# vita-epfl/collaborative-gan-sampling

Measured on AMD Instinct MI355X. Metric: refined samples/sec @ 20 refinement steps, higher is better.
Workload: dtype f32; 1 GPU; dcgan64 collaborative refinement (propose + K-step refine + render), batch 1024/GPU, K=20, momentum rate 0.1, refine at feature [8, 8, 256], random-init weights, z~U(-1,1) seed 2019+rank; global_batch=1024, refine_steps=20, parallelism=single GPU, hipgraph=True, batches_in_flight=2, fused_per_launch=1, sync_bn=False, contraction=f32

## Files before the change

collaborative-gan-sampling_amd/csrc/bn.hip:

```cpp
#include "cgs_internal.h"

#define BN_MAX_BLOCKS CGS_BN_MAX_BLOCKS

struct BnGeom {
    int G;
    int rows_per_block;
};

static BnGeom bn_geom(int M, int C) {
    BnGeom g;
    int rpb = cgs_ceil_div(M, BN_MAX_BLOCKS);
    if (rpb < 16) rpb = 16;
    g.rows_per_block = rpb;
    g.G = cgs_ceil_div(M, rpb);
    (void)C;
    return g;
}

size_t cgs_bn_ws_bytes(int M, int C) {
    (void)M;
    return ((size_t)BN_MAX_BLOCKS * 2 * C + 6 * (size_t)C) * sizeof(float);
}

__device__ __forceinline__ void bn_affine4(const float* __restrict__ mean, const float* __restrict__ invstd, const float* __restrict__ gamma,
// ... 388 lines not shown
        }
    }
    __syncthreads();
    if (!live) return;
    const float4 s0 = bc[0][q], s1 = bc[1][q];
    const int r0 = blockIdx.y * rows_per_block, r1 = min(M, r0 + rows_per_block);
    const size_t base = (size_t)grp * M * C + c;
    if (!BWD) {
        const float4 g = *(const float4*)(gamma + c), bt = *(const float4*)(beta + c);
        float4 sc, sh;
        sc.x = g.x * s1.x; sc.y = g.y * s1.y; sc.z = g.z * s1.z; sc.w = g.w * s1.w;
        sh.x = bt.x - s0.x * sc.x; sh.y = bt.y - s0.y * sc.y; sh.z = bt.z - s0.z * sc.z; sh.w = bt.w - s0.w * sc.w;
        for (int r = r0 + rl; r < r1; r += 16) {
            const float4 v = *(const float4*)(x + base + (size_t)r * C);
            float4 o;
            o.x = fmaf(v.x, sc.x, sh.x); o.y = fmaf(v.y, sc.y, sh.y); o.z = fmaf(v.z, sc.z, sh.z); o.w = fmaf(v.w, sc.w, sh.w);
            o.x = o.x > 0.f ? o.x : leak * o.x; o.y = o.y > 0.f ? o.y : leak * o.y;
            o.z = o.z > 0.f ? o.z : leak * o.z; o.w = o.w > 0.f ? o.w : leak * o.w;
            *(float4*)(out + base + (size_t)r * C) = o;
        }
    } else {
        float4 mean, inv, sc, sh;
        bn_affine4(mean_io + (size_t)grp * C, invstd_io + (size_t)grp * C, gamma, beta, c, mean, inv, sc, sh);
        const float4 m1 = s0, m2 = s1;
        for (int r = r0 + rl; r < r1; r += 16) {
            const float4 xv = *(const float4*)(x + base + (size_t)r * C), dv = *(const float4*)(dy + base + (size_t)r * C);
            float4 o;
            BWD1(x) BWD1(y) BWD1(z) BWD1(w)
            *(float4*)(out + base + (size_t)r * C) = o;
        }
    }
}

#undef BWD1

static int norm_fa_rows_per_block(int groups, int rows_per_seg, int nseg, int M_group, int C) {
    const long max_rows = 16;
    const size_t max_bytes = (size_t)2 << 20;
    if ((long)rows_per_seg * nseg > max_rows || (long)rows_per_seg * nseg > NFA_MAX_ROWS || groups > 65535) return 0;
    if ((size_t)groups * M_group * C * sizeof(float) > max_bytes) return 0;
    const long cg = cgs_ceil_div(C, 64);
    long chunks = 1024 / ((long)groups * cg);
    if (chunks < 1) chunks = 1;
    long rpb = cgs_ceil_div(M_group, (int)chunks);
    if (rpb < 16) rpb = 16;
    rpb = (rpb + 15) / 16 * 16;
    if (cgs_ceil_div(M_group, (int)rpb) > 65535) return 0;
    return (int)rpb;
}

int cgs_bn_train_lrelu_fwd(const float* x, const float* gamma, const float* beta, float eps, float leak, float* y,
                           float* mean, float* invstd, int M, int C, void* ws, size_t ws_bytes, void* stream) {
    if (M <= 0 || C <= 0 || (C & 3)) return cgs_set_error(CGS_EINVAL, "bn fwd: M=%d C=%d (C must be a multiple of 4)", M, C);
    if (ws_bytes < cgs_bn_ws_bytes(M, C)) return cgs_set_error(CGS_EWORKSPACE, "bn fwd: workspace %zu < %zu", ws_bytes, cgs_bn_ws_bytes(M, C));
    hipStream_t s = (hipStream_t)stream;
    if (norm_small_ok(M)) {
        hipLaunchKernelGGL(norm_small_kernel<false>, dim3(cgs_ceil_div(C, 64), 1), dim3(256), 0, s, x, nullptr, gamma, beta, eps, leak, y, mean, invstd, nullptr, M, C);
        CGS_CHECK_LAUNCH("bn_train_lrelu_fwd");
        return CGS_OK;
    }
    const BnGeom g = bn_geom(M, C);
    float* part = (float*)ws;
    float* stat = part + (size_t)BN_MAX_BLOCKS * 2 * C;
    hipLaunchKernelGGL(bn_partial_kernel<0>, dim3(g.G), dim3(256), 0, s, x, nullptr, nullptr, nullptr, nullptr, nullptr, leak, part, M, C, g.rows_per_block);
    hipLaunchKernelGGL(bn_finalize_kernel<0>, dim3(cgs_ceil_div(C, BNF_CH)), dim3(256), 0, s, part, g.G, M, C, gamma, beta, eps, stat, mean, invstd);
    const size_t n4 = (size_t)M * C / 4;
    hipLaunchKernelGGL(bn_apply_fwd_kernel, dim3(ew_blocks(n4)), dim3(256), 0, s, x, stat, leak, y, n4, C, n4);
    CGS_CHECK_LAUNCH("bn_train_lrelu_fwd");
// ... 237 lines not shown

int cgs_norm_lrelu_bwd_from_partials(const float* dy, const float* x, const float* part, int groups, int rows_per_seg, int nseg, int seg_stride,
                                     const float* gamma, const float* beta, const float* mean, const float* invstd, float leak, float* dx,
                                     int M_group, int C, void* ws, size_t ws_bytes, void* stream) {
    if (groups <= 0 || groups > 65535 || M_group <= 0 || C <= 0 || (C & 3) || rows_per_seg <= 0 || nseg <= 0 || seg_stride < 0 || !part || !dy || !x || !dx)
        return cgs_set_error(CGS_EINVAL, "norm bwd from partials: groups=%d M=%d C=%d rows=%d x %d", groups, M_group, C, rows_per_seg, nseg);
    const bool sliced = groups == 1 && nseg == 1 && rows_per_seg >= 1024 && !((uintptr_t)ws & 7);
    const size_t need = (size_t)groups * 2 * C * sizeof(float) + (sliced ? (size_t)BNF_SLICES * 2 * C * sizeof(double) : 0);
    if (!ws || ws_bytes < need) return cgs_set_error(CGS_EWORKSPACE, "norm bwd from partials: workspace %zu < %zu", ws_bytes, need);
    hipStream_t s = (hipStream_t)stream;
    if (const int rpb = norm_fa_rows_per_block(groups, rows_per_seg, nseg, M_group, C)) {
        hipLaunchKernelGGL(norm_fa_kernel<true>, dim3(cgs_ceil_div(C, 64), cgs_ceil_div(M_group, rpb), groups), dim3(256), 0, s, x, dy, part, rows_per_seg, nseg,
                           seg_stride, gamma, beta, 0.f, leak, dx, (float*)mean, (float*)invstd, M_group, C, rpb);
        CGS_CHECK_LAUNCH("norm_lrelu_bwd_from_partials");
        return CGS_OK;
    }
    float* stat2;
    if (sliced) {
        double* slices = (double*)ws;
        stat2 = (float*)(slices + (size_t)BNF_SLICES * 2 * C);
        hipLaunchKernelGGL(bn_slice_sums_kernel, dim3(cgs_ceil_div(C, BNF_CH), BNF_SLICES), dim3(256), 0, s, part, rows_per_seg, C, slices);
        hipLaunchKernelGGL(bn_finalize2_slices_kernel, dim3(cgs_ceil_div(C, 64)), dim3(64), 0, s, slices, M_group, C, stat2);
    } else {
        stat2 = (float*)ws;
        hipLaunchKernelGGL(bn_finalize_kernel<1>, dim3(cgs_ceil_div(C, BNF_CH), groups), dim3(256), 0, s, part, rows_per_seg, M_group, C, nullptr, nullptr, 0.f,
                           stat2, nullptr, nullptr, nseg, seg_stride);
    }
    const size_t n4 = (size_t)groups * M_group * C / 4, gn4 = (size_t)M_group * C / 4;
    hipLaunchKernelGGL(bn_apply_bwd_kernel, dim3(ew_blocks(n4)), dim3(256), 0, s, dy, x, mean, invstd, gamma, beta, stat2, leak, dx, n4, C, gn4);
    CGS_CHECK_LAUNCH("norm_lrelu_bwd_from_partials");
    return CGS_OK;
}

int cgs_instnorm_lrelu_bwd_data(const float* dy, const float* x, const float* scale, const float* offset, const float* mean,
                                const float* invstd, float leak, float* dx, int B, int HW, int C, void* ws, size_t ws_bytes,
                                void* stream) {
    if (B <= 0 || HW <= 0 || C <= 0 || (C & 3) || B > 65535) return cgs_set_error(CGS_EINVAL, "instnorm bwd: B=%d HW=%d C=%d", B, HW, C);
    if (ws_bytes < cgs_instnorm_ws_bytes(B, HW, C)) return cgs_set_error(CGS_EWORKSPACE, "instnorm bwd: workspace %zu < %zu", ws_bytes, cgs_instnorm_ws_bytes(B, HW, C));
    hipStream_t s = (hipStream_t)stream;
    const BnGeom g = in_geom(B, HW);
    float* part = (float*)ws;
    float* stat = part + (size_t)B * g.G * 2 * C;
    float* stat2 = stat + (size_t)B * 4 * C;
    if (norm_small_ok(HW)) {
        hipLaunchKernelGGL(norm_small_kernel<true>, dim3(cgs_ceil_div(C, 64), B), dim3(256), 0, s, x, dy, scale, offset, 0.f, leak, dx, (float*)mean, (float*)invstd, stat2, HW, C);
        CGS_CHECK_LAUNCH("instnorm_lrelu_bwd_data");
        return CGS_OK;
    }
    hipLaunchKernelGGL(bn_partial_kernel<1>, dim3(g.G, B), dim3(256), 0, s, x, dy, mean, invstd, scale, offset, leak, part, HW, C, g.rows_per_block);
    hipLaunchKernelGGL(bn_finalize_kernel<1>, dim3(cgs_ceil_div(C, BNF_CH), B), dim3(256), 0, s, part, g.G, HW, C, nullptr, nullptr, 0.f, stat2, nullptr, nullptr);
    const size_t n4 = (size_t)B * HW * C / 4, gn4 = (size_t)HW * C / 4;
    hipLaunchKernelGGL(bn_apply_bwd_kernel, dim3(ew_blocks(n4)), dim3(256), 0, s, dy, x, mean, invstd, scale, offset, stat2, leak, dx, n4, C, gn4);
    CGS_CHECK_LAUNCH("instnorm_lrelu_bwd_data");
    return CGS_OK;
}
```

collaborative-gan-sampling_amd/engine.py:

```python
import gc

import numpy as np
import torch

from . import kernels as K
from . import lib as L
from .nets import ARCHS, _same_out, g_input_shape, layer_ks


class _Stage:
    out = None
    bwd_epi = (L.EPI_NONE, None, None)
    pre_folded = False
    bwd_nstat = None
    bstat = None

    def fwd(self, x):
        raise NotImplementedError

    def bwd(self, dy):
        raise NotImplementedError


class _View(_Stage):
# ... 107 lines not shown
        return K.linear_bwd_data(dy, self.w, out=self.dx)


class _BnTrainLrelu(_Stage):

    def __init__(self, B, shape, gamma, beta, leak, dev):
        self.gamma, self.beta, self.leak = gamma, beta, leak
        self.out = torch.empty((B,) + tuple(shape), dtype=torch.float32, device=dev)
        self.mean = torch.empty(shape[-1], dtype=torch.float32, device=dev)
        self.invstd = torch.empty(shape[-1], dtype=torch.float32, device=dev)
        self.x = None

    sync = None
    groups = 1
    part = None

    part_layout = None

    def set_groups(self, groups, producer=None):
        self.groups = int(groups)
        self.part = self.part_layout = None
        if producer is not None:
            producer.part = producer.part_layout = None
            B = self.out.shape[0]
            self.part = producer.want_stats(B, B // self.groups)
            self.part_layout = producer.part_layout
        C = self.out.shape[-1]
        self.mean = torch.empty((self.groups, C), dtype=torch.float32, device=self.out.device)
        self.invstd = torch.empty((self.groups, C), dtype=torch.float32, device=self.out.device)

    def _g(self, t):
        return t.view(self.groups, -1, t.shape[-1])

    def fwd(self, x):
        self.x = x
        if self.bstat is not None:
            self.bstat.x = x
        if self.groups > 1:
            if self.part is not None:
                K.groupnorm_lrelu_fwd_from_partials(x, self.part, self.part_layout, self.groups, self.gamma, self.beta, self.leak,
                                                    out=self.out, stats=(self.mean, self.invstd))
            else:
                K.instnorm_lrelu_fwd(self._g(x), self.gamma, self.beta, self.leak, out=self._g(self.out), stats=(self.mean, self.invstd))
            return self.out
        if self.sync is None:
            if self.part is not None:
                K.bn_train_lrelu_fwd_from_partials(x, self.part, self.gamma, self.beta, self.leak, out=self.out, stats=(self.mean, self.invstd))
            else:
                K.bn_train_lrelu_fwd(x, self.gamma, self.beta, self.leak, out=self.out, stats=(self.mean, self.invstd))
            return self.out
        M = x.numel() // x.shape[-1]
        sums = self.sync.sums(x.shape[-1], x.device)
        K.bn_sync_fwd_sums(x, sums)
        self.sync.all_reduce(sums)
        K.bn_sync_fwd_apply(x, self.gamma, self.beta, sums, self.sync.world * M, self.leak, out=self.out,
                            stats=(self.mean, self.invstd))
        return self.out

    def bwd(self, dy):
        if self.bstat is not None:
            return K.norm_lrelu_bwd_from_partials(dy, self.x, self.bstat, self.groups, out=dy)
        if self.groups > 1:
            K.instnorm_lrelu_bwd_data(self._g(dy), self._g(self.x), self.gamma, self.beta, self.mean, self.invstd, self.leak,
                                      out=self._g(dy))
            return dy
        if self.sync is None:
            return K.bn_train_lrelu_bwd_data(dy, self.x, self.gamma, self.beta, self.mean, self.invstd, self.leak, out=dy)
# ... 328 lines not shown
                raise L.CgsError("bn_groups and sync_bn are mutually exclusive")

            def walk_g(stages):
                for below, st in zip([None] + stages[:-1], stages):
                    if isinstance(st, _BnTrainLrelu):
                        st.set_groups(self.bn_groups, below if isinstance(below, _Conv) else None)
                    if isinstance(st, _Residual):
                        walk_g(st.inner)
            walk_g(self.d.stages); walk_g(self.g_tail.stages)
        self.sync_bn = None
        if sync_bn is not None and sync_bn is not False:
            if use_graph:
                raise L.CgsError("sync_bn runs eagerly: the all-reduce between the two halves of a bn pass is not captured")
            self.sync_bn = BnSync(None if sync_bn is True else sync_bn)

            def walk(stages):
                for st in stages:
                    if isinstance(st, _BnTrainLrelu):
                        st.sync = self.sync_bn
                    if isinstance(st, _Residual):
                        walk(st.inner)
            walk(self.d.stages); walk(self.g_tail.stages)

        def drop_partials(stages):
            for below, st in zip([None] + stages[:-1], stages):
                if isinstance(st, _BnTrainLrelu) and st.sync is not None:
                    st.part = None
                    if isinstance(below, _Conv):
                        below.part = None
                if isinstance(st, _Residual):
                    drop_partials(st.inner)
        drop_partials(self.d.stages); drop_partials(self.g_tail.stages)
        link_norm_backward_stats(self.g_tail.stages + self.d.stages, B)

    def _sync_weights(self):
        if self._ws_epoch != K.WS.epoch:
            self._resync()

    def _resync(self):
        K.set_contraction(self.contraction)
        epoch = K.WS.epoch
        with torch.cuda.device(self.dev):
            for tape in (self.g_head, self.g_tail, self.d):
                for a, c, gamma, beta, mm, mv in tape.folds:
                    K.bn_fold(gamma, beta, mm, mv, out=(a, c))
            if self._gstream is not None and self._graphs:
                cur = torch.cuda.current_stream(self.dev)
                self._gstream.wait_stream(cur)
                with torch.cuda.stream(self._gstream):
                    self.forward_logits(self.theta, self.logit)
                    self.backward_to_feature()
                cur.wait_stream(self._gstream)
        self._ws_epoch = epoch

    @_entry
    def input_to_feature(self, z):
        self._sync_weights()
        return self.g_head.forward(z)

    @_entry
    def feature_to_data(self, feat):
        self._sync_weights()
        return self.g_tail.forward(feat)

    @_entry
    def discriminator(self, x):
        self._sync_weights()
        return self.d.forward(x)

    @_entry
    def generate(self, z):
        self._sync_weights()
        return self.g_tail.forward(self.g_head.forward(z))

    @_entry
    def score(self, images, out=None):
        self._sync_weights()
        return K.sigmoid_rowmean(self.d.forward(images), out=out)

    def forward_logits(self, theta, logit_out):
        x = self.g_tail.forward(theta)
        head = self.d.stages[-1]
        if isinstance(head, _Linear) and head.w.shape[1] == 1 and head.epi == L.EPI_NONE:
            for st in self.d.stages[:-1]:
                x = st.fwd(x)
            head.x_in = x
            return K.linear_out1_bce(x, head.w, head.b, head.out, self.dlogits, logit_out)
        logits = self.d.forward(x)
        K.bce_ones_grad_rowmean(logits, self.dlogits, logit_out)
        return logits

    def backward_to_feature(self):
        return self.g_tail.backward(self.d.backward(self.dlogits))

    @_entry
    def compute_forward_logits_and_grad(self, feature):
        self._sync_weights()
        self.forward_logits(feature, self.logit)
        return self.logit, self.backward_to_feature()

    def _program(self, steps, rate, alpha, probabilistic, vmin, vmax):
        th = self.theta
        render = self.g_tail.stages[-1].out
        self.forward_logits(th, self.logit)
        self.default_logit.copy_(self.logit)
        self.best_logit.copy_(self.logit)
        self.best_theta.copy_(th)
        self.images.copy_(render)
        self.best_step.fill_(1.0)
        self.tickets.zero_()
        forced = self.forced if probabilistic else None
        for i in range(steps):
            g = self.backward_to_feature()
            K.refine_update(th, self.mom, g, rate, alpha, first=(i == 0), vmin=vmin, vmax=vmax)
            self.forward_logits(th, self.logit)
            K.refine_select2(render, self.images, th, self.best_theta, self.logit, forced, i, self.best_logit, self.best_step, self.tickets)

    @_entry
    def refine(self, feature0, steps, rate, method="momentum", mode="deterministic", indices=None,
               vmin=None, vmax=None):
        if method == "momentum":
            alpha = 0.9
        elif method == "sgd":
            alpha = 0.0
        elif method == "ladam":
# ... 57 lines not shown
```

collaborative-gan-sampling_amd/kernels.py:

```python
import math
import weakref

import torch

from . import lib as L

LEAK = 0.2
BN_EPS = 1e-5


def _chk(t, name):
    if not (isinstance(t, torch.Tensor) and t.is_cuda and t.dtype == torch.float32 and t.is_contiguous()):
        raise L.CgsError(f"{name}: expected a contiguous fp32 tensor on the GPU, got "
                         f"{type(t).__name__} {getattr(t, 'dtype', None)} {getattr(t, 'device', None)}")
    return t


def _ptr(t):
    return None if t is None else t.data_ptr()


def _stream():
    return torch.cuda.current_stream().cuda_stream

# ... 447 lines not shown
        pr.done()
    return y, mean, invstd


def instnorm_lrelu_bwd_data(dy, x, scale, offset, mean, invstd, leak=1.0, out=None):
    _chk(dy, "dy"); _chk(x, "x")
    B, C = x.shape[0], x.shape[-1]
    HW = x.numel() // (B * C)
    dx = out if out is not None else torch.empty_like(x)
    ws = _in_workspace(B, HW, C, x.device)
    pr = _Prof(0.0, "", _nb(dy, x, dy, x, dx), op="instnorm_lrelu_bwd_data") if PROFILE is not None else None
    L.call("cgs_instnorm_lrelu_bwd_data", _ptr(dy), _ptr(x), _ptr(scale), _ptr(offset), _ptr(mean), _ptr(invstd), leak, _ptr(dx),
           B, HW, C, _ptr(ws), ws.numel() * 4, _stream())
    if pr is not None:
        pr.done()
    return dx


def norm_lrelu_bwd_from_partials(dy, x, nstat, groups, out=None):
    _chk(dy, "dy"); _chk(x, "x")
    C_ = x.shape[-1]
    Mg = x.numel() // (groups * C_)
    dx = out if out is not None else torch.empty_like(x)
    ws = _in_workspace(groups, Mg, C_, x.device) if groups > 1 else _bn_workspace(Mg, C_, x.device)
    lay = nstat.layout
    pr = _Prof(0.0, "", _nb(dy, x, dx), op="norm_lrelu_bwd_from_partials") if PROFILE is not None else None
    L.call("cgs_norm_lrelu_bwd_from_partials", _ptr(dy), _ptr(x), _ptr(nstat.part), groups, lay[1], lay[2], lay[3], _ptr(nstat.gamma), _ptr(nstat.beta),
           _ptr(nstat.mean), _ptr(nstat.invstd), nstat.leak, _ptr(dx), Mg, C_, _ptr(ws), ws.numel() * 4, _stream())
    if pr is not None:
        pr.done()
    return dx


def add(a, b, out=None):
    _chk(a, "a"); _chk(b, "b")
    o = out if out is not None else torch.empty_like(a)
    L.call("cgs_add", _ptr(a), _ptr(b), _ptr(o), a.numel(), _stream())
    return o


def bn_fold(gamma, beta, moving_mean, moving_var, eps=BN_EPS, out=None):
    C = gamma.numel()
    a, b = out if out is not None else (torch.empty(C, dtype=torch.float32, device=gamma.device),
                                        torch.empty(C, dtype=torch.float32, device=gamma.device))
    L.call("cgs_bn_fold", _ptr(gamma), _ptr(beta), _ptr(moving_mean), _ptr(moving_var), eps, _ptr(a), _ptr(b), C, _stream())
    return a, b


def affine_relu_fwd(x, a, b, out=None):
    _chk(x, "x")
    C = x.shape[-1]
    y = out if out is not None else torch.empty_like(x)
    L.call("cgs_affine_relu_fwd", _ptr(x), _ptr(a), _ptr(b), _ptr(y), x.numel() // C, C, _stream())
    return y


def affine_relu_bwd(dy, y, a, out=None):
    _chk(dy, "dy"); _chk(y, "y")
    C = y.shape[-1]
    dx = out if out is not None else torch.empty_like(y)
    L.call("cgs_affine_relu_bwd", _ptr(dy), _ptr(y), _ptr(a), _ptr(dx), y.numel() // C, C, _stream())
    return dx


def affine_fwd(x, a, b, out=None):
    _chk(x, "x")
# ... 190 lines not shown
```

collaborative-gan-sampling_amd/lib.py:

```python
import ctypes as C
import os

_HERE = os.path.dirname(os.path.abspath(__file__))
LIB_PATH = os.environ.get("CGS_LIB") or os.path.join(_HERE, "libcgs_hip.so")

OK, EINVAL, EWORKSPACE, ELAUNCH = 0, -1, -2, -3
EPI_NONE, EPI_LRELU, EPI_AFFINE_RELU, EPI_TANH = 0, 1, 2, 3
EPI_RELU_BWD_AFFINE, EPI_LRELU_BWD, EPI_TANH_BWD = 4, 5, 6
CONV_FWD, CONV_BWD_DATA, DECONV_FWD, DECONV_BWD_DATA = 0, 1, 2, 3
FAMILY_IGEMM, FAMILY_QUAD, FAMILY_SMALLN_T, FAMILY_SMALLN_F, FAMILY_PATCH, FAMILY_TAPS, FAMILY_DOT, FAMILY_IGEMM_BX6 = 0, 1, 2, 3, 4, 5, 6, 7
CONTRACTION_F32, CONTRACTION_BX6, CONTRACTION_BX6_ALL = 0, 1, 2
CONTRACTIONS = {"f32": CONTRACTION_F32, "bx6": CONTRACTION_BX6, "bx6_all": CONTRACTION_BX6_ALL}

_p, _i, _f, _z = C.c_void_p, C.c_int, C.c_float, C.c_size_t
_ll = C.c_longlong

SIGNATURES = {
    "cgs_version": (_i, []),
    "cgs_source_sha": (C.c_char_p, []),
    "cgs_last_error": (C.c_char_p, []),
    "cgs_last_kernel": (C.c_char_p, []),
    "cgs_last_executed_flops": (C.c_double, []),
    "cgs_last_tail_tiles": (_i, []),
    "cgs_last_tail_split": (_i, []),
    "cgs_set_contraction": (_i, [_i]),
    "cgs_get_contraction": (_i, []),
    "cgs_conv_ws_bytes": (_z, [_i] * 7),
    "cgs_conv_ws_bytes_for": (_z, [_i] * 10),
    "cgs_conv_family": (_i, [_i] * 13 + [_z]),
    "cgs_conv2d_nhwc_fwd": (_i, [_p] * 4 + [_i] * 9 + [_i, _p, _p, _p, _z, _i, _p]),
    "cgs_conv_stat_partials": (_i, [_i] * 9 + [_z]),
    "cgs_conv2d_nhwc_fwd_stats": (_i, [_p] * 4 + [_i] * 9 + [_p, _z, _i, _p, _z, _p]),
    "cgs_conv_stat_layout": (_i, [_i] * 13 + [_z, _p, _p, _p]),
    "cgs_deconv2d_nhwc_fwd_stats": (_i, [_p] * 4 + [_i] * 11 + [_p, _z, _i, _p, _z, _p]),
    "cgs_conv2d_nhwc_bwd_data_nstats": (_i, [_p] * 3 + [_i] * 9 + [_p] * 5 + [_f, _i, _p, _z, _i, _p, _z, _p]),
    "cgs_deconv2d_nhwc_bwd_data_nstats": (_i, [_p] * 3 + [_i] * 11 + [_p] * 5 + [_f, _i, _p, _z, _i, _p, _z, _p]),
    "cgs_norm_lrelu_bwd_from_partials": (_i, [_p] * 3 + [_i] * 4 + [_p] * 4 + [_f, _p, _i, _i, _p, _z, _p]),
    "cgs_groupnorm_lrelu_fwd_from_partials": (_i, [_p, _p, _i, _i, _i, _i, _p, _p, _f, _f, _p, _p, _p, _i, _i, _p, _z, _p]),
    "cgs_bn_train_lrelu_fwd_from_partials": (_i, [_p, _p, _i, _p, _p, _f, _f, _p, _p, _p, _i, _i, _p, _z, _p]),
    "cgs_conv2d_nhwc_bwd_data": (_i, [_p] * 3 + [_i] * 9 + [_i, _p, _p, _p, _z, _i, _p]),
    "cgs_deconv2d_nhwc_fwd": (_i, [_p] * 4 + [_i] * 11 + [_i, _p, _p, _p, _z, _i, _p]),
    "cgs_deconv2d_nhwc_bwd_data": (_i, [_p] * 3 + [_i] * 11 + [_i, _p, _p, _p, _z, _i, _p]),
    "cgs_conv_signs_ok": (_i, [_i] * 13 + [_z]),
    "cgs_deconv2d_nhwc_fwd_signs": (_i, [_p] * 4 + [_i] * 11 + [_i, _p, _p, _p, _p, _z, _i, _p]),
    "cgs_deconv2d_nhwc_bwd_data_signs": (_i, [_p] * 3 + [_i] * 11 + [_i, _p, _p, _p, _z, _i, _p]),
    "cgs_linear_fwd": (_i, [_p] * 4 + [_i] * 4 + [_p, _z, _i, _p]),
    "cgs_linear_bwd_data": (_i, [_p] * 3 + [_i] * 3 + [_p, _z, _i, _p]),
    "cgs_bn_ws_bytes": (_z, [_i, _i]),
    "cgs_bn_train_lrelu_fwd": (_i, [_p, _p, _p, _f, _f, _p, _p, _p, _i, _i, _p, _z, _p]),
    "cgs_bn_train_lrelu_bwd_data": (_i, [_p] * 6 + [_f, _p, _i, _i, _p, _z, _p]),
    "cgs_bn_sync_fwd_sums": (_i, [_p, _p, _i, _i, _p, _z, _p]),
    "cgs_bn_sync_fwd_apply": (_i, [_p, _p, _p, _f, _f, _p, _ll, _p, _p, _p, _i, _i, _p, _z, _p]),
    "cgs_bn_sync_bwd_sums": (_i, [_p] * 6 + [_f, _p, _i, _i, _p, _z, _p]),
    "cgs_bn_sync_bwd_apply": (_i, [_p] * 6 + [_f, _p, _ll, _p, _i, _i, _p, _z, _p]),
    "cgs_instnorm_ws_bytes": (_z, [_i, _i, _i]),
    "cgs_instnorm_lrelu_fwd": (_i, [_p, _p, _p, _f, _f, _p, _p, _p, _i, _i, _i, _p, _z, _p]),
    "cgs_instnorm_lrelu_bwd_data": (_i, [_p] * 6 + [_f, _p, _i, _i, _i, _p, _z, _p]),
    "cgs_add": (_i, [_p, _p, _p, _z, _p]),
    "cgs_bn_fold": (_i, [_p] * 4 + [_f, _p, _p, _i, _p]),
    "cgs_affine_relu_fwd": (_i, [_p] * 4 + [_i, _i, _p]),
    "cgs_affine_relu_bwd": (_i, [_p] * 4 + [_i, _i, _p]),
    "cgs_affine_fwd": (_i, [_p] * 4 + [_i, _i, _p]),
    "cgs_affine_bwd": (_i, [_p] * 3 + [_i, _i, _p]),
    "cgs_lrelu_fwd": (_i, [_p, _f, _p, _z, _p]),
    "cgs_lrelu_bwd": (_i, [_p, _p, _f, _p, _z, _p]),
    "cgs_tanh_fwd": (_i, [_p, _p, _z, _p]),
    "cgs_tanh_bwd": (_i, [_p, _p, _p, _z, _p]),
    "cgs_bce_ones_grad_rowmean": (_i, [_p, _p, _p, _i, _i, _p]),
    "cgs_bce_ones_fwd": (_i, [_p, _p, _z, _p]),
    "cgs_bce_ones_bwd": (_i, [_p, _p, _p, _z, _p]),
    "cgs_sigmoid_rowmean": (_i, [_p, _p, _i, _i, _p]),
    "cgs_clip": (_i, [_p, _f, _f, _p, _z, _p]),
    "cgs_refine_update": (_i, [_p, _p, _p, _f, _f, _i, _i, _f, _f, _z, _p]),
    "cgs_refine_select": (_i, [_p, _p, _p, _i, _p, _p, _p, _i, _i, _p]),
    "cgs_refine_select_rows": (_i, [_p, _p, _p, _i, _p, _p, _i, _i, _p]),
    "cgs_refine_select2": (_i, [_p, _p, _i, _p, _p, _i, _p, _p, _i, _p, _p, _p, _i, _p]),
    "cgs_linear_out1_bce": (_i, [_p, _p, _p, _p, _p, _p, _i, _i, _p]),
    "cgs_mlp2d_sigmoid_saliency": (_i, [_p, _p, _i, _i, _p, _p, _p, _i, _f, _p]),
    "cgs_refine2d": (_i, [_p, _p, _i, _i, _p, _f, _f, _i, _f, _i, _p, _p, _p, _i, _p]),
    "cgs_refine2d_devbase": (_i, [_p, _p, _i, _i, _p, _p, _f, _i, _f, _i, _p, _p, _p, _i, _p]),
    "cgs_mlp2d_train_ws_bytes": (_z, [_i, _i]),
    "cgs_mlp2d_d_step": (_i, [_p, _p, _i, _i, _p, _i, _p, _i, _f, _p, _p, _p, _p, _z, _p]),
    "cgs_mlp2d_gen_ws_bytes": (_z, [_i, _i, _i]),
# ... 113 lines not shown
```

include/cgs_hip.h:

```cpp
#ifndef CGS_HIP_H
#define CGS_HIP_H

#include <stddef.h>
#include <stdint.h>

#ifdef __cplusplus
extern "C" {
#endif

#define CGS_OK 0
#define CGS_EINVAL (-1)
#define CGS_EWORKSPACE (-2)
#define CGS_ELAUNCH (-3)

#define CGS_EPI_NONE 0
#define CGS_EPI_LRELU 1
#define CGS_EPI_AFFINE_RELU 2
#define CGS_EPI_TANH 3
#define CGS_EPI_RELU_BWD_AFFINE 4
#define CGS_EPI_LRELU_BWD 5
#define CGS_EPI_TANH_BWD 6

#define CGS_CONV_FWD 0
#define CGS_CONV_BWD_DATA 1
// ... 74 lines not shown
                               int B, int H, int W, int Cin, int Ho, int Wo, int Cout, int kh, int kw, int sh, int sw,
                               int epilogue, const float* ep_a, const float* ep_aux,
                               void* ws, size_t ws_bytes, int ws_prepacked, void* stream);

int cgs_conv_signs_ok(int op, int B, int H, int W, int Cin, int Ho, int Wo, int Cout, int kh, int kw, int sh, int sw,
                      int epilogue, size_t ws_bytes);
int cgs_deconv2d_nhwc_fwd_signs(const float* x, const float* w, const float* bias, float* y,
                                int B, int H, int W, int Cin, int Ho, int Wo, int Cout, int kh, int kw, int sh, int sw,
                                int epilogue, const float* ep_a, const float* ep_b, unsigned* signs,
                                void* ws, size_t ws_bytes, int ws_prepacked, void* stream);
int cgs_deconv2d_nhwc_bwd_data_signs(const float* dy, const float* w, float* dx,
                                     int B, int H, int W, int Cin, int Ho, int Wo, int Cout, int kh, int kw, int sh, int sw,
                                     int epilogue, const float* ep_a, const unsigned* aux_signs,
                                     void* ws, size_t ws_bytes, int ws_prepacked, void* stream);

int cgs_linear_fwd(const float* x, const float* w, const float* bias, float* y, int B, int in, int out,
                   int epilogue, void* ws, size_t ws_bytes, int ws_prepacked, void* stream);
int cgs_linear_out1_bce(const float* x, const float* w, const float* bias, float* logits, float* dlogits, float* logit_mean, int B, int in,
                        void* stream);
int cgs_linear_bwd_data(const float* dy, const float* w, float* dx, int B, int in, int out,
                        void* ws, size_t ws_bytes, int ws_prepacked, void* stream);

size_t cgs_bn_ws_bytes(int M, int C);
int cgs_bn_train_lrelu_fwd(const float* x, const float* gamma, const float* beta, float eps, float leak,
                           float* y, float* mean, float* invstd, int M, int C,
                           void* ws, size_t ws_bytes, void* stream);
int cgs_bn_train_lrelu_fwd_from_partials(const float* x, const float* part, int G, const float* gamma, const float* beta,
                                         float eps, float leak, float* y, float* mean, float* invstd, int M, int C,
                                         void* ws, size_t ws_bytes, void* stream);
int cgs_bn_train_lrelu_bwd_data(const float* dy, const float* x, const float* gamma, const float* beta,
                                const float* mean, const float* invstd, float leak, float* dx, int M, int C,
                                void* ws, size_t ws_bytes, void* stream);

int cgs_bn_sync_fwd_sums(const float* x, double* sums, int M, int C, void* ws, size_t ws_bytes, void* stream);
int cgs_bn_sync_fwd_apply(const float* x, const float* gamma, const float* beta, float eps, float leak, const double* sums,
                          long long M_total, float* y, float* mean, float* invstd, int M, int C,
                          void* ws, size_t ws_bytes, void* stream);
int cgs_bn_sync_bwd_sums(const float* dy, const float* x, const float* gamma, const float* beta, const float* mean,
                         const float* invstd, float leak, double* sums, int M, int C, void* ws, size_t ws_bytes, void* stream);
int cgs_bn_sync_bwd_apply(const float* dy, const float* x, const float* gamma, const float* beta, const float* mean,
                          const float* invstd, float leak, const double* sums, long long M_total, float* dx, int M, int C,
                          void* ws, size_t ws_bytes, void* stream);

size_t cgs_instnorm_ws_bytes(int B, int HW, int C);
int cgs_instnorm_lrelu_fwd(const float* x, const float* scale, const float* offset, float eps, float leak, float* y,
                           float* mean, float* invstd, int B, int HW, int C, void* ws, size_t ws_bytes, void* stream);
int cgs_instnorm_lrelu_bwd_data(const float* dy, const float* x, const float* scale, const float* offset,
                                const float* mean, const float* invstd, float leak, float* dx, int B, int HW, int C,
                                void* ws, size_t ws_bytes, void* stream);
int cgs_groupnorm_lrelu_fwd_from_partials(const float* x, const float* part, int groups, int rows_per_seg, int nseg, int seg_stride,
                                          const float* gamma, const float* beta, float eps, float leak, float* y, float* mean,
                                          float* invstd, int M_group, int C, void* ws, size_t ws_bytes, void* stream);
int cgs_add(const float* a, const float* b, float* out, size_t n, void* stream);

int cgs_bn_fold(const float* gamma, const float* beta, const float* moving_mean, const float* moving_var,
                float eps, float* a, float* b, int C, void* stream);
int cgs_affine_relu_fwd(const float* x, const float* a, const float* b, float* y, int M, int C, void* stream);
int cgs_affine_relu_bwd(const float* dy, const float* y, const float* a, float* dx, int M, int C, void* stream);
int cgs_affine_fwd(const float* x, const float* a, const float* b, float* y, int M, int C, void* stream);
int cgs_affine_bwd(const float* dy, const float* a, float* dx, int M, int C, void* stream);
int cgs_lrelu_fwd(const float* x, float leak, float* y, size_t n, void* stream);
int cgs_lrelu_bwd(const float* dy, const float* y, float leak, float* dx, size_t n, void* stream);
int cgs_tanh_fwd(const float* x, float* y, size_t n, void* stream);
int cgs_tanh_bwd(const float* dy, const float* y, float* dx, size_t n, void* stream);

int cgs_bce_ones_grad_rowmean(const float* logits, float* dlogits, float* logit_mean, int B, int P, void* stream);
// ... 54 lines not shown
```

Before: 6658 samples/s.

## Fuse final BN+LeakyReLU with discriminator linear head in forward and backward

Adds HIP kernels that fold the last batch-norm + LeakyReLU of the discriminator into the 1-output linear head. The normalized activation tensor is never written in the forward pass, and the backward pass recomputes the head gradient and normalization backward in place from x and dlogits. This removes a full activation write and read plus separate linear-head launches on every refinement step. The BN output is materialized lazily through a property only if something else reads it. The cost is extra recomputation in the backward kernels and more complex stage bookkeeping.

```diff
diff --git a/collaborative-gan-sampling_amd/csrc/bn.hip b/collaborative-gan-sampling_amd/csrc/bn.hip
--- a/collaborative-gan-sampling_amd/csrc/bn.hip
+++ b/collaborative-gan-sampling_amd/csrc/bn.hip
@@ -444,8 +444,6 @@
     }
 }
 
-#undef BWD1
-
 static int norm_fa_rows_per_block(int groups, int rows_per_seg, int nseg, int M_group, int C) {
     const long max_rows = 16;
     const size_t max_bytes = (size_t)2 << 20;
@@ -749,6 +747,222 @@
     return CGS_OK;
 }
 
+#define HEAD1(f, xv, ww)                                                     \
+        {                                                                    \
+            float a = fmaf(xv.f, sc.f, sh.f);                                \
+            a = a > 0.f ? a : leak * a;                                      \
+            s = fmaf(a, ww.f, s);                                            \
+        }
+__global__ __launch_bounds__(256) void bn_head_fwd_kernel(const float* __restrict__ x, const float* __restrict__ stat0 ,
+                                                          const float* __restrict__ w, const float* __restrict__ bias, float leak,
+                                                          float* __restrict__ y, float* __restrict__ dl, float* __restrict__ lm,
+                                                          int B, int K, int C, int group_B) {
+    const int b = blockIdx.x * 4 + (threadIdx.x >> 6);
+    const int lane = threadIdx.x & 63;
+    if (b >= B) return;
+    const float* row = x + (size_t)b * K;
+    const float* scale = stat0 + (size_t)(b / group_B) * 4 * C + 2 * C;
+    const float* shift = scale + C;
+    float s = 0.f;
+    int k = lane * 4;
+    for (; k + 3 * 256 < K; k += 4 * 256) {
+        const float4 x0 = *(const float4*)(row + k), x1 = *(const float4*)(row + k + 256), x2 = *(const float4*)(row + k + 512),
+                     x3 = *(const float4*)(row + k + 768);
+#define HEADQ(xq, off)                                                                                  \
+        {                                                                                               \
+            const int c = (k + off) % C;                                                                \
+            const float4 sc = *(const float4*)(scale + c), sh = *(const float4*)(shift + c);            \
+            const float4 ww = *(const float4*)(w + k + off);                                            \
+            HEAD1(x, xq, ww) HEAD1(y, xq, ww) HEAD1(z, xq, ww) HEAD1(w, xq, ww)                         \
+        }
+        HEADQ(x0, 0) HEADQ(x1, 256) HEADQ(x2, 512) HEADQ(x3, 768)
+    }
+    for (; k < K; k += 256) {
+        const float4 x0 = *(const float4*)(row + k);
+        HEADQ(x0, 0)
+    }
+#undef HEADQ
+#pragma unroll
+    for (int off = 32; off > 0; off >>= 1) s += __shfl_down(s, off, 64);
+    if (lane == 0) {
+        const float v = s + (bias ? bias[0] : 0.f);
+        y[b] = v;
+        dl[b] = v >= 0.f ? -expf(-v) / (1.f + expf(-v)) : -1.f / (1.f + expf(v));
+        lm[b] = v;
+    }
+}
+#undef HEAD1
+
+__global__ __launch_bounds__(256) void bn_head_bwd_sums_kernel(const float* __restrict__ x, const float* __restrict__ dl, const float* __restrict__ w,
+                                                               const float* __restrict__ mean_p, const float* __restrict__ invstd_p,
+                                                               const float* __restrict__ gamma, const float* __restrict__ beta, float leak,
+                                                               float* __restrict__ part, int K, int C, int HW, int group_B, int chunk_B) {
+    __shared__ float4 red[2][4][64];
+    const int q = threadIdx.x & 63, sl = threadIdx.x >> 6;
+    const int k = (blockIdx.x * 64 + q) * 4;
+    const int grp = blockIdx.z;
+    const bool live = k < K;
+    float4 sa = make_float4(0.f, 0.f, 0.f, 0.f), sb = sa;
+    int p = 0, c = 0;
+    if (live) {
+        p = k / C; c = k - p * C;
+        float4 mean, inv, sc, sh;
+        bn_affine4(mean_p + (size_t)grp * C, invstd_p + (size_t)grp * C, gamma, beta, c, mean, inv, sc, sh);
+        const float4 ww = *(const float4*)(w + k);
+        const int b0 = grp * group_B + blockIdx.y * chunk_B;
+        const int b1 = min(b0 + chunk_B, (grp + 1) * group_B);
+#pragma unroll 4
+        for (int b = b0 + sl; b < b1; b += 4) {
+            const float4 xv = *(const float4*)(x + (size_t)b * K + k);
+            const float g = dl[b];
+#define HS1(f)                                                                          \
+            {                                                                           \
+                const float dv = g * ww.f;                                              \
+                const float u = fmaf(xv.f, sc.f, sh.f);                                 \
+                const float d = dv * (u > 0.f ? 1.f : leak);                            \
+                sa.f += d; sb.f = fmaf(d, (xv.f - mean.f) * inv.f, sb.f);               \
+            }
+            HS1(x) HS1(y) HS1(z) HS1(w)
+#undef HS1
+        }
+    }
+    red[0][sl][q] = sa; red[1][sl][q] = sb;
+    __syncthreads();
+    if (sl != 0 || !live) return;
+    float4 ta = red[0][0][q], tb = red[1][0][q];
+    for (int i = 1; i < 4; ++i) {
+        const float4 a = red[0][i][q], b = red[1][i][q];
+        ta.x += a.x; ta.y += a.y; ta.z += a.z; ta.w += a.w;
+        tb.x += b.x; tb.y += b.y; tb.z += b.z; tb.w += b.w;
+    }
+    float* rowp = part + (((size_t)grp * gridDim.y + blockIdx.y) * HW + p) * 2 * C;
+    *(float4*)(rowp + c) = ta;
+    *(float4*)(rowp + C + c) = tb;
+}
+
+__global__ __launch_bounds__(256) void bn_head_bwd_apply_kernel(const float* __restrict__ x, const float* __restrict__ dl, const float* __restrict__ w,
+                                                                const float* __restrict__ mean_p, const float* __restrict__ invstd_p,
+                                                                const float* __restrict__ gamma, const float* __restrict__ beta,
+                                                                const float* __restrict__ stat20 , float leak,
+                                                                float* __restrict__ dx, int K, int C, int group_B, int chunk_B) {
+    const int k = (blockIdx.x * 256 + threadIdx.x) * 4;
+    if (k >= K) return;
+    const int grp = blockIdx.z;
+    const int c = k % C;
+    float4 mean, inv, sc, sh;
+    bn_affine4(mean_p + (size_t)grp * C, invstd_p + (size_t)grp * C, gamma, beta, c, mean, inv, sc, sh);
+    const float4 m1 = *(const float4*)(stat20 + (size_t)grp * 2 * C + c), m2 = *(const float4*)(stat20 + (size_t)grp * 2 * C + C + c);
+    const float4 ww = *(const float4*)(w + k);
+    const int b0 = grp * group_B + blockIdx.y * chunk_B;
+    const int b1 = min(b0 + chunk_B, (grp + 1) * group_B);
+#pragma unroll 4
+    for (int b = b0; b < b1; ++b) {
+        const float4 xv = *(const float4*)(x + (size_t)b * K + k);
+        const float g = dl[b];
+        float4 dv, o;
+        dv.x = g * ww.x; dv.y = g * ww.y; dv.z = g * ww.z; dv.w = g * ww.w;
+        BWD1(x) BWD1(y) BWD1(z) BWD1(w)
+        *(float4*)(dx + (size_t)b * K + k) = o;
+    }
+}
+#undef BWD1
+
+struct HeadGeom {
+    int fwd_G;
+    int fwd_rpb;
+    int chunk_B;
+    int chunks;
+    int apply_B;
+};
+
+static HeadGeom head_geom(int B, int HW, int C, int groups) {
+    HeadGeom g;
+    const int group_B = B / groups;
+    const BnGeom f = groups == 1 ? bn_geom(group_B * HW, C) : in_geom(groups, group_B * HW);
+    g.fwd_G = f.G; g.fwd_rpb = f.rows_per_block;
+    int max_rows = 2048 / groups;
+    if (max_rows > BN_MAX_BLOCKS) max_rows = BN_MAX_BLOCKS;
+    int chunks = max_rows / HW;
+    if (chunks < 1) chunks = 1;
+    int cb = cgs_ceil_div(group_B, chunks);
+    cb = (cb + 3) / 4 * 4;
+    g.chunk_B = cb;
+    g.chunks = cgs_ceil_div(group_B, cb);
+    const long xb = cgs_ceil_div(HW * C / 4, 256);
+    g.apply_B = xb * groups * cgs_ceil_div(group_B, 8) >= 1024 ? 8 : 2;
+    return g;
+}
+
+static bool head_args_ok(int B, int HW, int C, int groups) {
+    return B > 0 && HW > 0 && C > 0 && !(C & 3) && groups > 0 && groups <= 65535 && B % groups == 0 && (long long)HW * C <= 0x7fffffff / 4 &&
+           (long long)B * HW <= 0x7fffffff;
+}
+
+size_t cgs_bn_head_ws_bytes(int B, int HW, int C, int groups) {
+    if (!head_args_ok(B, HW, C, groups)) return 0;
+    const HeadGeom g = head_geom(B, HW, C, groups);
+    const int rows = g.fwd_G > g.chunks * HW ? g.fwd_G : g.chunks * HW;
+    size_t area = (size_t)groups * rows * 2 * C * sizeof(float);
+    const size_t slices = (size_t)BNF_SLICES * 2 * C * sizeof(double);
+    if (area < slices) area = slices;
+    return area + (size_t)groups * 6 * C * sizeof(float);
+}
+
+int cgs_bn_head_bwd_rows(int B, int HW, int C, int groups) {
+    return head_args_ok(B, HW, C, groups) ? head_geom(B, HW, C, groups).chunks * HW : 0;
+}
+
+int cgs_bn_head_fwd(const float* x, const float* part, int rows_per_seg, int nseg, int seg_stride, int groups, const float* gamma,
+                    const float* beta, float eps, float leak, const float* w, const float* bias, float* logits, float* dlogits,
+                    float* logit_mean, float* mean, float* invstd, int B, int HW, int C, void* ws, size_t ws_bytes, void* stream) {
+    if (!head_args_ok(B, HW, C, groups) || !x || !gamma || !beta || !w || !logits || !dlogits || !logit_mean || !mean || !invstd ||
+        (part && (rows_per_seg <= 0 || nseg <= 0 || seg_stride < 0)))
+        return cgs_set_error(CGS_EINVAL, "bn head fwd: B=%d HW=%d C=%d groups=%d rows=%d x %d", B, HW, C, groups, rows_per_seg, nseg);
+    const size_t need = cgs_bn_head_ws_bytes(B, HW, C, groups);
+    if (!ws || ((uintptr_t)ws & 15) || ws_bytes < need) return cgs_set_error(CGS_EWORKSPACE, "bn head fwd: workspace %zu < %zu (16-byte aligned)", ws_bytes, need);
+    hipStream_t s = (hipStream_t)stream;
+    const HeadGeom g = head_geom(B, HW, C, groups);
+    const int group_B = B / groups, Mg = group_B * HW;
+    float* stat = (float*)((char*)ws + need) - (size_t)groups * 6 * C;
+    if (!part) {
+        float* own = (float*)ws;
+        hipLaunchKernelGGL(bn_partial_kernel<0>, dim3(g.fwd_G, groups), dim3(256), 0, s, x, nullptr, nullptr, nullptr, nullptr, nullptr, leak, own, Mg, C, g.fwd_rpb);
+        hipLaunchKernelGGL(bn_finalize_kernel<0>, dim3(cgs_ceil_div(C, BNF_CH), groups), dim3(256), 0, s, own, g.fwd_G, Mg, C, gamma, beta, eps, stat, mean, invstd);
+    } else if (groups == 1 && nseg == 1 && rows_per_seg >= 1024) {
+        double* slices = (double*)ws;
+        hipLaunchKernelGGL(bn_slice_sums_kernel, dim3(cgs_ceil_div(C, BNF_CH), BNF_SLICES), dim3(256), 0, s, part, rows_per_seg, C, slices);
+        hipLaunchKernelGGL(bn_finalize_slices_kernel, dim3(cgs_ceil_div(C, 64)), dim3(64), 0, s, slices, Mg, C, gamma, beta, eps, stat, mean, invstd);
+    } else {
+        hipLaunchKernelGGL(bn_finalize_kernel<0>, dim3(cgs_ceil_div(C, BNF_CH), groups), dim3(256), 0, s, part, rows_per_seg, Mg, C, gamma, beta, eps, stat,
+                           mean, invstd, nseg, seg_stride);
+    }
+    hipLaunchKernelGGL(bn_head_fwd_kernel, dim3(cgs_ceil_div(B, 4)), dim3(256), 0, s, x, stat, w, bias, leak, logits, dlogits, logit_mean, B, HW * C, C, group_B);
+    CGS_CHECK_LAUNCH("bn_head_fwd");
+    return CGS_OK;
+}
+
+int cgs_bn_head_bwd_data(const float* dlogits, const float* w, const float* x, const float* gamma, const float* beta, const float* mean,
+                         const float* invstd, float leak, float* dx, int groups, int B, int HW, int C, void* ws, size_t ws_bytes,
+                         void* stream) {
+    if (!head_args_ok(B, HW, C, groups) || !dlogits || !w || !x || !gamma || !beta || !mean || !invstd || !dx)
+        return cgs_set_error(CGS_EINVAL, "bn head bwd: B=%d HW=%d C=%d groups=%d", B, HW, C, groups);
+    const size_t need = cgs_bn_head_ws_bytes(B, HW, C, groups);
+    if (!ws || ((uintptr_t)ws & 15) || ws_bytes < need) return cgs_set_error(CGS_EWORKSPACE, "bn head bwd: workspace %zu < %zu (16-byte aligned)", ws_bytes, need);
+    hipStream_t s = (hipStream_t)stream;
+    const HeadGeom g = head_geom(B, HW, C, groups);
+    const int group_B = B / groups, K = HW * C, G = g.chunks * HW;
+    float* part = (float*)ws;
+    float* stat2 = (float*)((char*)ws + need) - (size_t)groups * 2 * C;
+    hipLaunchKernelGGL(bn_head_bwd_sums_kernel, dim3(cgs_ceil_div(K / 4, 64), g.chunks, groups), dim3(256), 0, s, x, dlogits, w, mean, invstd, gamma, beta, leak,
+                       part, K, C, HW, group_B, g.chunk_B);
+    hipLaunchKernelGGL(bn_finalize_kernel<1>, dim3(cgs_ceil_div(C, BNF_CH), groups), dim3(256), 0, s, part, G, group_B * HW, C, nullptr, nullptr, 0.f, stat2,
+                       nullptr, nullptr);
+    hipLaunchKernelGGL(bn_head_bwd_apply_kernel, dim3(cgs_ceil_div(K / 4, 256), cgs_ceil_div(group_B, g.apply_B), groups), dim3(256), 0, s, x, dlogits, w, mean,
+                       invstd, gamma, beta, stat2, leak, dx, K, C, group_B, g.apply_B);
+    CGS_CHECK_LAUNCH("bn_head_bwd_data");
+    return CGS_OK;
+}
+
 int cgs_instnorm_lrelu_bwd_data(const float* dy, const float* x, const float* scale, const float* offset, const float* mean,
                                 const float* invstd, float leak, float* dx, int B, int HW, int C, void* ws, size_t ws_bytes,
                                 void* stream) {
diff --git a/collaborative-gan-sampling_amd/engine.py b/collaborative-gan-sampling_amd/engine.py
--- a/collaborative-gan-sampling_amd/engine.py
+++ b/collaborative-gan-sampling_amd/engine.py
@@ -163,7 +163,27 @@
     def _g(self, t):
         return t.view(self.groups, -1, t.shape[-1])
 
-    def fwd(self, x):
+    out_skipped = False
+
+    @property
+    def out(self):
+        if self.out_skipped:
+            self.out_skipped = False
+            C = self._out.shape[-1]
+            scratch = (torch.empty((self.groups, C), dtype=torch.float32, device=self._out.device),
+                       torch.empty((self.groups, C), dtype=torch.float32, device=self._out.device))
+            if self.groups > 1:
+                K.instnorm_lrelu_fwd(self._g(self.x), self.gamma, self.beta, self.leak, out=self._g(self._out), stats=scratch)
+            else:
+                K.bn_train_lrelu_fwd(self.x, self.gamma, self.beta, self.leak, out=self._out, stats=(scratch[0].view(-1), scratch[1].view(-1)))
+        return self._out
+
+    @out.setter
+    def out(self, t):
+        self._out = t
+
+    def fwd(self, x):
+        self.out_skipped = False
         self.x = x
         if self.bstat is not None:
             self.bstat.x = x
@@ -558,6 +578,23 @@
                     drop_partials(st.inner)
         drop_partials(self.d.stages); drop_partials(self.g_tail.stages)
         link_norm_backward_stats(self.g_tail.stages + self.d.stages, B)
+        self.fused_head = self._find_fused_head()
+
+    def _find_fused_head(self):
+        st = self.d.stages
+        if not (st and isinstance(st[-1], _Linear) and st[-1].w.shape[1] == 1 and st[-1].epi == L.EPI_NONE):
+            return None
+        n = len(st) - 2
+        if n >= 0 and isinstance(st[n], _View):
+            n -= 1
+        if n < 1 or not isinstance(st[n], _BnTrainLrelu):
+            return None
+        bn = st[n]
+        if bn.sync is not None or bn.part is None or bn.bstat is not None or st[n - 1].part_layout is None:
+            return None
+        if bn.out[0].numel() != st[-1].w.shape[0]:
+            return None
+        return n, bn, st[-1]
 
     def _sync_weights(self):
         if self._ws_epoch != K.WS.epoch:
@@ -607,6 +644,14 @@
     def forward_logits(self, theta, logit_out):
         x = self.g_tail.forward(theta)
         head = self.d.stages[-1]
+        if self.fused_head is not None:
+            n, bn, head = self.fused_head
+            for st in self.d.stages[:n]:
+                x = st.fwd(x)
+            bn.x = x
+            bn.out_skipped = True
+            return K.bn_head_fwd(x, bn.gamma, bn.beta, head.w, head.b, head.out, self.dlogits, logit_out, (bn.mean, bn.invstd),
+                                 groups=bn.groups, part=bn.part, layout=self.d.stages[n - 1].part_layout, leak=bn.leak)
         if isinstance(head, _Linear) and head.w.shape[1] == 1 and head.epi == L.EPI_NONE:
             for st in self.d.stages[:-1]:
                 x = st.fwd(x)
@@ -617,6 +662,13 @@
         return logits
 
     def backward_to_feature(self):
+        if self.fused_head is not None:
+            n, bn, head = self.fused_head
+            dy = K.bn_head_bwd_data(self.dlogits, head.w, bn.x, bn.gamma, bn.beta, bn.mean, bn.invstd, groups=bn.groups, leak=bn.leak,
+                                    out=head.dx.view(bn.x.shape))
+            for st in reversed(self.d.stages[:n]):
+                dy = st.bwd(dy)
+            return self.g_tail.backward(dy)
         return self.g_tail.backward(self.d.backward(self.dlogits))
 
     @_entry
diff --git a/collaborative-gan-sampling_amd/kernels.py b/collaborative-gan-sampling_amd/kernels.py
--- a/collaborative-gan-sampling_amd/kernels.py
+++ b/collaborative-gan-sampling_amd/kernels.py
@@ -503,6 +503,52 @@
     return dx
 
 
+_head_ws = {}
+
+
+def _head_workspace(B, HW, C, groups, device):
+    key = (B, HW, C, groups, device.index, torch.cuda.current_stream(device).cuda_stream)
+    ws = _head_ws.get(key)
+    if ws is None:
+        nbytes = int(L.load().cgs_bn_head_ws_bytes(B, HW, C, groups))
+        if nbytes == 0:
+            raise L.CgsError(f"bn head: B={B} HW={HW} C={C} groups={groups} (C must be a multiple of 4, groups must divide B)")
+        ws = torch.empty(nbytes // 4, dtype=torch.float32, device=device)
+        _head_ws[key] = ws
+    return ws
+
+
+def bn_head_fwd(x, gamma, beta, w, bias, logits, dlogits, logit_mean, stats, groups=1, part=None, layout=None, leak=LEAK, eps=BN_EPS):
+    _chk(x, "x"); _chk(w, "w")
+    B, C = x.shape[0], x.shape[-1]
+    HW = x.numel() // (B * C)
+    if w.numel() != HW * C:
+        raise L.CgsError(f"bn head: weight of {w.numel()} elements for rows of {HW * C}")
+    mean, invstd = stats
+    ws = _head_workspace(B, HW, C, groups, x.device)
+    lay = layout if part is not None else (0, 0, 0, 0)
+    pr = _Prof(2.0 * B * HW * C, "", _nb(x, w, logits), op="bn_head_fwd") if PROFILE is not None else None
+    L.call("cgs_bn_head_fwd", _ptr(x), _ptr(part), lay[1], lay[2], lay[3], groups, _ptr(gamma), _ptr(beta), eps, leak, _ptr(w), _ptr(bias),
+           _ptr(logits), _ptr(dlogits), _ptr(logit_mean), _ptr(mean), _ptr(invstd), B, HW, C, _ptr(ws), ws.numel() * 4, _stream())
+    if pr is not None:
+        pr.done()
+    return logits
+
+
+def bn_head_bwd_data(dlogits, w, x, gamma, beta, mean, invstd, groups=1, leak=LEAK, out=None):
+    _chk(x, "x"); _chk(w, "w"); _chk(dlogits, "dlogits")
+    B, C = x.shape[0], x.shape[-1]
+    HW = x.numel() // (B * C)
+    dx = out if out is not None else torch.empty_like(x)
+    ws = _head_workspace(B, HW, C, groups, x.device)
+    pr = _Prof(0.0, "", _nb(x, x, dx), op="bn_head_bwd_data") if PROFILE is not None else None
+    L.call("cgs_bn_head_bwd_data", _ptr(dlogits), _ptr(w), _ptr(x), _ptr(gamma), _ptr(beta), _ptr(mean), _ptr(invstd), leak, _ptr(dx),
+           groups, B, HW, C, _ptr(ws), ws.numel() * 4, _stream())
+    if pr is not None:
+        pr.done()
+    return dx
+
+
 def add(a, b, out=None):
     _chk(a, "a"); _chk(b, "b")
     o = out if out is not None else torch.empty_like(a)
diff --git a/collaborative-gan-sampling_amd/lib.py b/collaborative-gan-sampling_amd/lib.py
--- a/collaborative-gan-sampling_amd/lib.py
+++ b/collaborative-gan-sampling_amd/lib.py
@@ -49,6 +49,10 @@
     "cgs_bn_ws_bytes": (_z, [_i, _i]),
     "cgs_bn_train_lrelu_fwd": (_i, [_p, _p, _p, _f, _f, _p, _p, _p, _i, _i, _p, _z, _p]),
     "cgs_bn_train_lrelu_bwd_data": (_i, [_p] * 6 + [_f, _p, _i, _i, _p, _z, _p]),
+    "cgs_bn_head_ws_bytes": (_z, [_i] * 4),
+    "cgs_bn_head_bwd_rows": (_i, [_i] * 4),
+    "cgs_bn_head_fwd": (_i, [_p, _p, _i, _i, _i, _i, _p, _p, _f, _f] + [_p] * 7 + [_i, _i, _i, _p, _z, _p]),
+    "cgs_bn_head_bwd_data": (_i, [_p] * 7 + [_f, _p, _i, _i, _i, _i, _p, _z, _p]),
     "cgs_bn_sync_fwd_sums": (_i, [_p, _p, _i, _i, _p, _z, _p]),
     "cgs_bn_sync_fwd_apply": (_i, [_p, _p, _p, _f, _f, _p, _ll, _p, _p, _p, _i, _i, _p, _z, _p]),
     "cgs_bn_sync_bwd_sums": (_i, [_p] * 6 + [_f, _p, _i, _i, _p, _z, _p]),
diff --git a/include/cgs_hip.h b/include/cgs_hip.h
--- a/include/cgs_hip.h
+++ b/include/cgs_hip.h
@@ -130,6 +130,16 @@
                                 const float* mean, const float* invstd, float leak, float* dx, int M, int C,
                                 void* ws, size_t ws_bytes, void* stream);
 
+size_t cgs_bn_head_ws_bytes(int B, int HW, int C, int groups);
+int cgs_bn_head_bwd_rows(int B, int HW, int C, int groups);
+int cgs_bn_head_fwd(const float* x, const float* part, int rows_per_seg, int nseg, int seg_stride, int groups,
+                    const float* gamma, const float* beta, float eps, float leak, const float* w, const float* bias,
+                    float* logits, float* dlogits, float* logit_mean, float* mean, float* invstd, int B, int HW, int C,
+                    void* ws, size_t ws_bytes, void* stream);
+int cgs_bn_head_bwd_data(const float* dlogits, const float* w, const float* x, const float* gamma, const float* beta,
+                         const float* mean, const float* invstd, float leak, float* dx, int groups, int B, int HW, int C,
+                         void* ws, size_t ws_bytes, void* stream);
+
 int cgs_bn_sync_fwd_sums(const float* x, double* sums, int M, int C, void* ws, size_t ws_bytes, void* stream);
 int cgs_bn_sync_fwd_apply(const float* x, const float* gamma, const float* beta, float eps, float leak, const double* sums,
                           long long M_total, float* y, float* mean, float* invstd, int M, int C,
```

After: 6690 samples/s (median of 6 runs). About the same (+0.5%).
